# wanxinjin/Pontryagin-Differentiable-Programming

Measured on AMD Instinct MI355X. Metric: trajectories/sec (fwd+Riccati+PDP grad), quadrotor n=13 T=50, higher is better.
Workload: dtype f64

## Files before the change

pontryagin-differentiable-programming_amd/csrc/pdp_fused3_kernels.h:

```cpp
#pragma once
#include "pdp_model_kernels.h"
#include "pdp_wave.h"

#ifndef PDP_F3_GAIN_AHEAD
#define PDP_F3_GAIN_AHEAD 3
#endif
#ifndef PDP_F3_ROLLOUT_LANES
#define PDP_F3_ROLLOUT_LANES 0
#endif

namespace pdp {

#ifdef PDP_PHASE_TIMING
__device__ long long g_rb_stamp[16];
#endif

template <class Mdl, int XW = 0>
struct Fused3Layout {
    using L = FusedLayout<Mdl>;
    static constexpr int NX = Mdl::NX, NU = Mdl::NU, NP = Mdl::NP;
    static constexpr int NCB = 1 + Mdl::PATHA_NCONST + Mdl::PATHB_NCONST, NCF = 1 + Mdl::FWD_NCONST, NCFIN = 1 + Mdl::FIN_NCONST;
    static constexpr int NA = Mdl::PATHA_NVAR, NB = Mdl::PATHB_NVAR > 16 ? Mdl::PATHB_NVAR : 16;
    static constexpr int CB0 = NA + NB;
    static constexpr int BSTRIDE = (CB0 + NCB) | 1;
// ... 79 lines not shown
    long long ts[12]; int nts = 0; long long twait = 0, tw0 = 0;
    const long long rt0 = __builtin_amdgcn_s_memrealtime();
    for (int i = 0; i < 12; ++i) ts[i] = 0;
#define F3_STAMP() ts[nts++] = __builtin_readcyclecounter()
#define F3_W0() tw0 = __builtin_readcyclecounter()
#define F3_W1() twait += __builtin_readcyclecounter() - tw0
#else
#define F3_STAMP()
#define F3_W0()
#define F3_W1()
#endif
    F3_STAMP();

    if (runner) {
        __builtin_amdgcn_s_setprio(3);
        {
            double th0[NP], pc0[Mdl::NPC];
            load_theta<Mdl>(theta, b, tb, th0);
            Mdl::precompute(th0, pc0);
            if (lane == 0) {
#pragma unroll
                for (int i = 0; i < NP; ++i) par[i] = th0[i];
#pragma unroll
                for (int i = 0; i < Mdl::NPC; ++i) par[NP + i] = pc0[i];
            }
            wg_signal(fl + 0, 1);
        }
        double xTr[NX];
        if (given) {
#pragma unroll
            for (int i = 0; i < NX; ++i) xTr[i] = xb[T * NX + i];
        } else {
            double* us = pool;
            for (int i = lane; i < T * NU; i += 64) us[i] = ub[i];
            PDP_F3_PAR();
            double xc[NX], xn[NX], uc[NU];
#pragma unroll
            for (int i = 0; i < NX; ++i) xc[i] = x0[(int64_t)b * NX + i];
            if (lane == 0) {
#pragma unroll
                for (int i = 0; i < NX; ++i) xb[i] = xc[i];
            }
            wave_lds_sync();
            const auto rsX = PDP_BUF_RSRC(xb, (T + 1) * NX * 8);
            const unsigned xvoff = lane == 0 ? 0u : BUF_OOB;
            double un[NU];
#pragma unroll
            for (int i = 0; i < NU; ++i) un[i] = us[i];
#if PDP_F3_ROLLOUT_LANES
            double xs[NX];
#pragma unroll
            for (int i = 0; i < NX; ++i) xs[i] = 0.0;
            for (int tb_ = 0; tb_ < T; tb_ += 64) {
                const int nb = min(64, T - tb_);
                for (int tl_ = 0; tl_ < nb; ++tl_) {
                    const int t = tb_ + tl_, tn = t + 1 < T ? t + 1 : t;
#pragma unroll
                    for (int i = 0; i < NU; ++i) { uc[i] = un[i]; un[i] = us[tn * NU + i]; }
                    Mdl::dyn(xc, uc, th, pc, xn);
                    const bool mine = lane == tl_;
#pragma unroll
                    for (int i = 0; i < NX; ++i) { xc[i] = xn[i]; xs[i] = mine ? xn[i] : xs[i]; }
                }
                const unsigned vo = lane < nb ? (unsigned)(lane * NX) * 8u : BUF_OOB;
                const unsigned so = (unsigned)((tb_ + 1) * NX) * 8u;
#pragma unroll
                for (int i = 0; i + 1 < NX; i += 2) buf_store_f64x2(rsX, so, vo + 8u * i, xs[i], xs[i + 1]);
                if constexpr (NX & 1) buf_store_f64(rsX, so, vo + 8u * (NX - 1), xs[NX - 1]);
            }
#else
            for (int t = 0; t < T; ++t) {
                const int tn = t + 1 < T ? t + 1 : t;
#pragma unroll
                for (int i = 0; i < NU; ++i) { uc[i] = un[i]; un[i] = us[tn * NU + i]; }
                Mdl::dyn(xc, uc, th, pc, xn);
#pragma unroll
                for (int i = 0; i < NX; ++i) xc[i] = xn[i];
                {
                    const unsigned so = (unsigned)((t + 1) * NX) * 8u;
#pragma unroll
                    for (int i = 0; i + 1 < NX; i += 2) buf_store_f64x2(rsX, so, xvoff + 8u * i, xn[i], xn[i + 1]);
                    if constexpr (NX & 1) buf_store_f64(rsX, so, xvoff + 8u * (NX - 1), xn[NX - 1]);
                }
            }
#endif
#pragma unroll
            for (int i = 0; i < NX; ++i) xTr[i] = xc[i];
        }
        wg_signal(fl + 0, 2);
        F3_STAMP();

        bool ok = true;
        d4 P, W2;
        {
            if (lane == 0) fin[0] = 0.0;
            for (int i_ = lane; i_ < Mdl::FIN_NCONST; i_ += 64) fin[1 + i_] = Mdl::fin_const(i_);
            if (lane == 0) {
                PDP_F3_PAR();
                PackedSink s{fin + F3::NCFIN};
                Mdl::eval_fin(xTr, nullptr, nullptr, th, pc, s);
            }
            wave_lds_sync();
            Gather gP, gW;
            make_gather(gP, lane, F3::NCFIN, 0, [](int r, int c) { return (r < NX && c < NX) ? Mdl::fin_code(0, r * NX + c) : -1; });
            make_gather(gW, lane, F3::NCFIN, 0, [](int r, int c) { return (r < NX && c >= M && c < M + NP) ? Mdl::fin_code(1, r * NP + (c - M)) : -1; });
            P = gather_tile(fin, gP, 0);
            W2 = gather_tile(fin, gW, 0);
        }
        F3_STAMP();

        {
            constexpr int NA = F3::NA, NCA = Mdl::PATHA_NCONST;
            auto codeA = [](int mat, int i) { return Mdl::patha_code(mat, i); };
            auto codeB = [](int mat, int i) { int c = Mdl::pathb_code(mat, i); return c >= 0 ? c + NA : (c == -1 ? -1 : c - NCA); };
            RowGather gF, gY, gHxx, gHX, gHU, gGr, gHux;
            make_row_gather(gF, lane, F3::CB0, [&](int r, int c) { return (r < NX && c < NX) ? codeA(0, r * NX + c) : -1; });
            make_row_gather(gY, lane, F3::CB0, [&](int r, int c) {
                return r >= NX ? -1 : (c < M ? codeA(1, r * NU + c) : (c < M + NP ? codeA(2, r * NP + (c - M)) : -1)); });
            make_row_gather(gGr, lane, F3::CB0, [&](int r, int c) { return (r < NX && (c & 3) < NU) ? codeA(1, r * NU + (c & 3)) : -1; });
            make_row_gather(gHux, lane, F3::CB0, [&](int r, int c) { return (r < M && c < NX) ? codeB(1, c * NU + r) : -1; });
            make_row_gather(gHxx, lane, F3::CB0, [&](int r, int c) { return (r < NX && c < NX) ? codeB(0, r * NX + c) : -1; });
            make_row_gather(gHX, lane, F3::CB0, [&](int r, int c) {
                return r >= NX ? -1 : (c < M ? codeB(1, r * NU + c) : (c < M + NP ? codeB(2, r * NP + (c - M)) : -1)); });
            make_row_gather(gHU, lane, F3::CB0, [&](int r, int c) {
                return r >= M ? -1 : (c < M ? codeB(3, r * NU + c) : (c < M + NP ? codeB(4, r * NP + (c - M)) : -1)); });
            const TileMapBytes mK = make_tile_map_sink(NU, NX, NX, 0, 0, lane, GSZ0 - 1), mIK = make_tile_map_sink(NU, NP, NP, 0, M, lane, NU * NP);
            constexpr int RSZ = oc_riccati_doubles<Mdl>();
            [[maybe_unused]] const BufMap mRP = f3_store_map(NX, NX, NX, 0, lane), mRW = f3_store_map(NX, NP, NP, M, lane);
            [[maybe_unused]] const auto rsR = PDP_BUF_RSRC(FM::RIC && riccati ? riccati + (int64_t)b * T * RSZ : ws_gain, FM::RIC && riccati ? (int64_t)T * RSZ * 8 : 0);
            [[maybe_unused]] const PredMaps<Mdl> pm(lane);
            [[maybe_unused]] const bool precPW = FM::RIC && prec && !(flags & PDP_OC_RECORD_PRIMAL);
            [[maybe_unused]] const auto rsPR = PDP_BUF_RSRC(precPW ? (void*)(prec + (int64_t)b * T * PredRec<Mdl>::SIZE) : (void*)ws_gain, precPW ? (int64_t)T * PredRec<Mdl>::SIZE * 4 : 0);
            constexpr int RB = 8 * BS;
            for (int g = 0; g < nchunk; ++g) {
                int t0, cnt;
                bchunk(g, t0, cnt);
                const double* pb = pool + (g & 1) * F3::BUF;
                F3_W0();
                wg_wait_ge(fl + 2, g + 1);
                F3_W1();
                int tl = cnt - 1;
                const double* r0 = pb + (tl - 1) * BS;
                RowRun rF = row_run_at(gF, r0), rY = row_run_at(gY, r0), rHxx = row_run_at(gHxx, r0), rHX = row_run_at(gHX, r0), rHU = row_run_at(gHU, r0),
                     rGr = row_run_at(gGr, r0), rHux = row_run_at(gHux, r0);
                auto move_all = [&](int bytes) {
                    row_move(rF, bytes); row_move(rY, bytes); row_move(rHxx, bytes); row_move(rHX, bytes); row_move<1>(rHU, bytes); row_move(rGr, bytes); row_move<1>(rHux, bytes);
                };
                d4 Fa = row_read(rF, RB), Ya = row_read(rY, RB), Fb = z, Yb = z;
                auto bstep = [&](int tl, unsigned imm, const d4 Fc, const d4 Yc, d4& Fn, d4& Yn) {
                    const int t = t0 + tl;
#ifdef PDP_PHASE_TIMING_FINE
                    if (blockIdx.x == 0 && threadIdx.x == 0) g_rb_stamp[9] = __builtin_readcyclecounter();
#endif
                    d4 Hxx = row_read(rHxx, imm), HX2 = row_read(rHX, imm), HU2 = row_read<1>(rHU, imm), Grep = row_read(rGr, imm), Hux = row_read<1>(rHux, imm);
                    if (tl > 0) { Fn = row_read(rF, imm - RB); Yn = row_read(rY, imm - RB); }
                    RiccatiGains gn;
                    d4 P_old;
                    if constexpr (FM::RIC) {
                        if (riccati) { buf_store(rsR, (unsigned)(t * RSZ) * 8u, mRP, P); buf_store(rsR, (unsigned)(t * RSZ + NX * NX) * 8u, mRW, W2); }
                        if (precPW) { pred_store(rsPR, (unsigned)(t * PredRec<Mdl>::SIZE) * 4u, pm.P, P); pred_store(rsPR, (unsigned)(t * PredRec<Mdl>::SIZE) * 4u, pm.W, W2); }
                    }
                    ok = riccati_backward<M, false>(P, W2, Fc, Yc, Grep, Hxx, HX2, HU2, Hux[0], scratch, lane, NP, gn, P_old) && ok;
                    store_all<1>(gw + t * GSZ, mK, gn.K);
                    store_all<1>(gw + t * GSZ + NX * NU, mIK, gn.IK);
#ifdef PDP_PHASE_TIMING_FINE
                    if (blockIdx.x == 0 && threadIdx.x == 0) { g_rb_stamp[11] = g_rb_stamp[10]; g_rb_stamp[10] = __builtin_readcyclecounter(); }
#endif
                };
                for (; (tl + 1) % U != 0; --tl) { bstep(tl, RB, Fa, Ya, Fb, Yb); Fa = Fb; Ya = Yb; move_all(-RB); }
                move_all(-(U - 1) * RB);
                for (; tl >= U - 1; tl -= U) {
                    static_assert(U == 4, "the group is written out");
                    bstep(tl, (unsigned)(4 * RB), Fa, Ya, Fb, Yb);
                    bstep(tl - 1, (unsigned)(3 * RB), Fb, Yb, Fa, Ya);
                    bstep(tl - 2, (unsigned)(2 * RB), Fa, Ya, Fb, Yb);
                    bstep(tl - 3, (unsigned)(1 * RB), Fb, Yb, Fa, Ya);
                    move_all(-U * RB);
                }
                wg_signal(fl + 3, g + 1);
            }
        }
        bool finite = tile_finite(P) && tile_finite(W2);
        F3_STAMP();

        double acc = 0.0;
        [[maybe_unused]] double lsum = 0.0;
        double dT;
        [[maybe_unused]] bool obsT = true;
        [[maybe_unused]] double sT = 0.0, rhoT = 0.0;
        if constexpr (FM::WLS) { const int li = lane < NX ? lane : 0; wls_slot(dT, sT, xb[T * NX + li], dxb[T * NX + li], wxb[T * NX + li], oc_wls_x(oc_wls(wls...)), rhoT); }
        else if constexpr (FM::COT) dT = lane < NX ? dxb[T * NX + lane] : 0.0;
        else if constexpr (FM::MISS) { const double dd = lane < NX ? dxb[T * NX + lane] : 0.0; obsT = dd == dd; dT = lane < NX ? (obsT ? xb[T * NX + lane] - dd : dd) : 0.0; }
        else dT = lane < NX ? xb[T * NX + lane] - dxb[T * NX + lane] : 0.0;
        d4 X2 = z;
        [[maybe_unused]] d4 Gn = z;
        {
            constexpr int DLX = Mdl::FWD_NVAR, DLU = Mdl::FWD_NVAR + NX;
            [[maybe_unused]] constexpr int DSX = DLU + NU, DSU = DSX + NX;
            RowGather gFT, gGT, gE, gDX, gDU;
            [[maybe_unused]] RowGather gSX, gSU;
            if constexpr (FM::WLS) {
                make_row_gather(gSX, lane, F3::CF0, [](int r, int c) { return (r < NX) ? DSX + r : -1; });
                make_row_gather(gSU, lane, F3::CF0, [](int r, int c) { return (r < M) ? DSU + r : -1; });
            }
            make_row_gather(gFT, lane, F3::CF0, [](int r, int c) { return (r < NX && c < NX) ? Mdl::fwd_code(0, c * NX + r) : -1; });
            make_row_gather(gGT, lane, F3::CF0, [](int r, int c) { return (r < M && c < NX) ? Mdl::fwd_code(1, c * NU + r) : -1; });
            make_row_gather(gE, lane, F3::CF0, [](int r, int c) { return (r < NX && c >= M && c < M + NP) ? Mdl::fwd_code(2, r * NP + (c - M)) : -1; });
            make_row_gather(gDX, lane, F3::CF0, [](int r, int c) { return (r < NX) ? DLX + r : -1; });
            make_row_gather(gDU, lane, F3::CF0, [](int r, int c) { return (r < M) ? DLU + r : -1; });
            const TileMapBytes mKT = to_bytes_sink(make_rep4_map_transposed(NX, NU, NX, lane), GSZ0 - 1), mIK = make_tile_map_sink(NU, NP, NP, 0, M, lane, NU * NP);
#if PDP_F3_GAIN_AHEAD >= 2
            d4 KTs[4], ks[4];
#pragma unroll
            for (int s_ = 0; s_ < 4; ++s_) {
                if (s_ < PDP_F3_GAIN_AHEAD) {
                    const int ts = s_ < T ? s_ : T - 1;
                    KTs[s_] = -load_all<4>(gw + ts * GSZ, mKT);
                    ks[s_] = -load_all<1>(gw + ts * GSZ + NX * NU, mIK);
                } else { KTs[s_] = z; ks[s_] = z; }
            }
#else
            d4 KTn = -load_all<4>(gw, mKT);
            d4 kn = -load_all<1>(gw + NX * NU, mIK);
#endif
            [[maybe_unused]] const BufMap mSX = f3_store_map(NX, NP, NP, M, lane), mSU = f3_store_map(NU, NP, NP, M, lane);
            [[maybe_unused]] const auto rsSX = PDP_BUF_RSRC(dxdp ? dxdp + (int64_t)b * (T + 1) * NX * NP : ws_gain, dxdp ? (int64_t)(T + 1) * NX * NP * 8 : 0);
            [[maybe_unused]] const auto rsSU = PDP_BUF_RSRC(dudp ? dudp + (int64_t)b * T * NU * NP : ws_gain, dudp ? (int64_t)T * NU * NP * 8 : 0);
            [[maybe_unused]] const PredMaps<Mdl> pmf(lane);
            [[maybe_unused]] const auto rsPRf = PDP_BUF_RSRC(FM::RIC && prec ? (void*)(prec + (int64_t)b * T * PredRec<Mdl>::SIZE) : (void*)ws_gain, FM::RIC && prec ? (int64_t)T * PredRec<Mdl>::SIZE * 4 : 0);
            constexpr int RF = 8 * FS;
            static_assert((U & 1) == 0, "the register sets of the unrolled loops alternate: U must be even");
            for (int c = 0; c < nchunkF; ++c) {
                const int g = nchunk + c, t0 = c * chF, cnt = min(chF, T - t0);
                const double* pb = pool + (g & 1) * F3::BUF;
                F3_W0();
                wg_wait_ge(fl + 2, g + 1);
                F3_W1();
                RowRun rFT = row_run_at(gFT, pb), rGT = row_run_at(gGT, pb), rE = row_run_at(gE, pb), rDX = row_run_at(gDX, pb), rDU = row_run_at(gDU, pb);
                [[maybe_unused]] RowRun rSX, rSU;
                if constexpr (FM::WLS) { rSX = row_run_at(gSX, pb); rSU = row_run_at(gSU, pb); }
                auto move_all = [&](int bytes) {
                    row_move(rFT, bytes); row_move<1>(rGT, bytes); row_move(rE, bytes); row_move(rDX, bytes); row_move<1>(rDU, bytes);
                    if constexpr (FM::WLS) { row_move(rSX, bytes); row_move<1>(rSU, bytes); }
                };
                auto fstep = [&](int tl, unsigned imm, const d4 Xc, d4& Xn, const d4 KTc, const d4 kc, d4& KTnx, d4& knx) {
                    const int t = t0 + tl, tnx = (t + PDP_F3_GAIN_AHEAD < T) ? t + PDP_F3_GAIN_AHEAD : T - 1;
                    KTnx = -load_all<4>(gw + tnx * GSZ, mKT);
                    knx = -load_all<1>(gw + tnx * GSZ + NX * NU, mIK);
                    d4 FT = row_read(rFT, imm);
                    d4 GT = row_read<1>(rGT, imm);
                    d4 E2 = row_read(rE, imm);
                    d4 DX = row_read(rDX, imm);
                    d4 DU = row_read<1>(rDU, imm);
                    d4 U2;
                    riccati_forward(KTc, kc, FT, GT, E2, Xc, U2, Xn);
                    d4 Xm = Xc, Um = U2;
                    if constexpr (FM::WLS) {
                        const d4 SX = row_read(rSX, imm), SU = row_read<1>(rSU, imm);
                        Xm = wls_scale(SX, Xc);
                        Um = zero4(); Um[0] = wls_scale(SU, U2)[0];
                    } else
                    mask_step<FM::MISS, 4>(DX, DU, Xc, U2, Xm, Um);
                    if constexpr (FM::GN) Gn = gram_step<false>(Xm, Um, Gn);
                    acc += contract_step(DX, DU, Xm, Um);
                    if constexpr (FM::RIC) {
                        if (dxdp || dudp) {
                            buf_store(rsSX, (unsigned)(t * NX * NP) * 8u, mSX, Xc);
                            buf_store<1>(rsSU, (unsigned)(t * NU * NP) * 8u, mSU, U2);
                        }
                        if (prec) {
                            pred_store(rsPRf, (unsigned)(t * PredRec<Mdl>::SIZE) * 4u, pmf.X, Xn);
                            pred_store<1>(rsPRf, (unsigned)(t * PredRec<Mdl>::SIZE) * 4u, pmf.U, U2);
                        }
                    } else {
                        if (dxdp) store_dense(dxdp + ((int64_t)b * (T + 1) + t) * NX * NP, NX, NP, NP, 0, M, lane, Xc);
                        if (dudp) store_dense(dudp + ((int64_t)b * T + t) * NU * NP, NU, NP, NP, 0, M, lane, U2);
                    }
                };
                d4 Xb;
                int tl = 0;
#if PDP_F3_GAIN_AHEAD >= 2
                static_assert(U == 4 && PDP_F3_GAIN_AHEAD <= 3, "four gain sets rotate through a group of four steps");
                constexpr int A = PDP_F3_GAIN_AHEAD;
                for (; tl + U <= cnt; tl += U) {
                    fstep(tl + 0, (unsigned)(0 * RF), X2, Xb, KTs[0], ks[0], KTs[(0 + A) & 3], ks[(0 + A) & 3]);
                    fstep(tl + 1, (unsigned)(1 * RF), Xb, X2, KTs[1], ks[1], KTs[(1 + A) & 3], ks[(1 + A) & 3]);
                    fstep(tl + 2, (unsigned)(2 * RF), X2, Xb, KTs[2], ks[2], KTs[(2 + A) & 3], ks[(2 + A) & 3]);
                    fstep(tl + 3, (unsigned)(3 * RF), Xb, X2, KTs[3], ks[3], KTs[(3 + A) & 3], ks[(3 + A) & 3]);
                    move_all(U * RF);
                }
                for (; tl < cnt; ++tl) {
                    fstep(tl, 0u, X2, Xb, KTs[0], ks[0], KTs[A], ks[A]);
                    X2 = Xb;
#pragma unroll
                    for (int s_ = 0; s_ < A; ++s_) { KTs[s_] = KTs[s_ + 1]; ks[s_] = ks[s_ + 1]; }
                    move_all(RF);
                }
#else
                d4 KTb, kb;
                for (; tl + U <= cnt; tl += U) {
#pragma unroll
                    for (int j = 0; j < U; ++j) {
                        if (j & 1) fstep(tl + j, (unsigned)(j * RF), Xb, X2, KTb, kb, KTn, kn);
                        else fstep(tl + j, (unsigned)(j * RF), X2, Xb, KTn, kn, KTb, kb);
                    }
                    move_all(U * RF);
                }
                for (; tl < cnt; ++tl) { fstep(tl, 0u, X2, Xb, KTn, kn, KTb, kb); X2 = Xb; KTn = KTb; kn = kb; move_all(RF); }
#endif
                wg_signal(fl + 3, g + 1);
            }
        }
        F3_STAMP();
        wave_lds_sync();
        if (lane < NX) {
// ... 207 lines not shown
```

pontryagin-differentiable-programming_amd/csrc/pdp_riccati.h:

```cpp
#pragma once
#include "pdp_tile.h"

namespace pdp {

constexpr int RICCATI_SCRATCH = 272 + 272 + 64;

PDP_DEV void tile_to_lds17(double* s, const d4 v, int lane) {
#pragma unroll
    for (int r = 0; r < 4; ++r) s[tile_row(lane, r) * 17 + tile_col(lane)] = v[r];
}
PDP_DEV d4 tile_from_lds17_transposed(const double* s, int lane) {
    d4 v;
#pragma unroll
    for (int r = 0; r < 4; ++r) v[r] = s[tile_col(lane) * 17 + tile_row(lane, r)];
    return v;
}

struct RiccatiGains {
    d4 KT;
    d4 K;
    d4 IK;
    d4 Z;
    double Zrep;
    d4 Qux;
    bool pd;
};

template <int M>
PDP_DEV bool posdef_small(const double* a) {
    if constexpr (M == 1) return a[0] > 0.0;
    else if constexpr (M == 2) return a[0] > 0.0 && a[0] * a[3] - a[1] * a[2] > 0.0;
    else {
        const double d2 = a[0] * a[4] - a[1] * a[3];
        const double d3 = a[0] * (a[4] * a[8] - a[5] * a[7]) - a[1] * (a[3] * a[8] - a[5] * a[6]) + a[2] * (a[3] * a[7] - a[4] * a[6]);
        return a[0] > 0.0 && d2 > 0.0 && d3 > 0.0;
    }
}

#ifndef PDP_RB_T
#define PDP_RB_T(i)
#endif
template <int M, bool WANT_KT = true, bool HUX_FROM_HX2 = false, bool WANT_PD = false>
PDP_DEV bool riccati_backward(d4& P, d4& W0, const d4 Ft, const d4 Y2, const d4 Grep, const d4 Hxx, const d4 HX2, const d4 HU2, double Hux0,
                              double* scratch, int lane, int p0, RiccatiGains& g, d4& P_old_out) {
    const d4 z = zero4();
    if constexpr (HUX_FROM_HX2) tile_to_lds17(scratch, HX2, lane);
    PDP_RB_T(0);
    d4 PF = mma_tn(P, Ft, z);
    d4 PY2 = mma_tn(P, Y2, W0);
    PDP_RB_T(1);
    d4 FY = mma_tn(Ft, PY2, HX2);
    d4 Q2 = z;
    Q2[0] = mma4_tn(Grep, PY2, HU2[0]);
    PDP_RB_T(2);
    if constexpr (HUX_FROM_HX2) {
        wave_lds_sync();
        Hux0 = ((lane >> 4) < M) ? scratch[(lane & 15) * 17 + (lane >> 4)] : 0.0;
    }
    d4 Qux = z;
    Qux[0] = mma4_tn(Grep, PF, Hux0);
    d4 Pn = mma_tn(Ft, PF, Hxx);
    P_old_out = P;
    PDP_RB_T(3);
    const int row = lane >> 4, col = lane & 15;
    d4 Z = z;
    double Zrep = 0.0;
    bool ok = true;
    if constexpr (M == 4) {
        scratch[544 + lane] = Q2[0];
        wave_lds_sync();
        PDP_RB_T(4);
        const int i = row, j = col & 3;
        const int r0 = (i == 0) ? 1 : 0, r1 = (i <= 1) ? 2 : 1, r2 = (i <= 2) ? 3 : 2;
        const int c0 = (j == 0) ? 1 : 0, c1 = (j <= 1) ? 2 : 1, c2 = (j <= 2) ? 3 : 2;
        const double* q = scratch + 544;
        const double m00 = q[r0 * 16 + c0], m01 = q[r0 * 16 + c1], m02 = q[r0 * 16 + c2];
        const double m10 = q[r1 * 16 + c0], m11 = q[r1 * 16 + c1], m12 = q[r1 * 16 + c2];
        const double m20 = q[r2 * 16 + c0], m21 = q[r2 * 16 + c1], m22 = q[r2 * 16 + c2];
        double cof = m00 * (m11 * m22 - m12 * m21) - m01 * (m10 * m22 - m12 * m20) + m02 * (m10 * m21 - m11 * m20);
        cof = ((i + j) & 1) ? -cof : cof;
        const double ac = Q2[0] * cof;
        const double t0 = readlane_f64(ac, 0), t1 = readlane_f64(ac, 1), t2 = readlane_f64(ac, 2), t3 = readlane_f64(ac, 3);
        const double det = (t0 + t1) + (t2 + t3), mag = (fabs(t0) + fabs(t1)) + (fabs(t2) + fabs(t3));
        if constexpr (WANT_PD) {
            const double a00 = readlane_f64(Q2[0], 0), a01 = readlane_f64(Q2[0], 1), a10 = readlane_f64(Q2[0], 16), a11 = readlane_f64(Q2[0], 17);
            g.pd = a00 > 0.0 && a00 * a11 - a01 * a10 > 0.0 && readlane_f64(cof, 51) > 0.0 && det > 0.0;
        }
        if (fabs(det) > COFACTOR4_GUARD * mag && fabs(det) <= 1.7e308) {
            double rdet = __builtin_amdgcn_rcp(det);
            rdet = fma(fma(-det, rdet, 1.0), rdet, rdet);
            Zrep = cof * rdet;
        } else {
            double a[16], ai[16];
#pragma unroll
            for (int ii = 0; ii < 4; ++ii)
#pragma unroll
                for (int jj = 0; jj < 4; ++jj) a[ii * 4 + jj] = readlane_f64(Q2[0], 16 * ii + jj);
            ok = inverse_small<4>(a, ai);
            double zz = 0.0;
#pragma unroll
            for (int ii = 0; ii < 4; ++ii)
#pragma unroll
                for (int jj = 0; jj < 4; ++jj) zz = (row == ii && (col & 3) == jj) ? ai[jj * 4 + ii] : zz;
            Zrep = zz;
        }
    } else {
        double a[M * M], ai[M * M];
#pragma unroll
        for (int i = 0; i < M; ++i)
#pragma unroll
            for (int j = 0; j < M; ++j) a[i * M + j] = readlane_f64(Q2[0], 16 * i + j);
        ok = inverse_small_fast<M>(a, ai);
        if constexpr (WANT_PD) g.pd = posdef_small<M>(a);
        double zz = 0.0;
#pragma unroll
        for (int i = 0; i < M; ++i)
#pragma unroll
            for (int j = 0; j < M; ++j) zz = (row == i && (col & 3) == j) ? ai[j * M + i] : zz;
        Zrep = zz;
    }
    Z[0] = (col < 4) ? Zrep : 0.0;
    PDP_RB_T(5);
    d4 K = z;
    K[0] = mma4_blk(Zrep, Qux[0], 0.0);
    g.IK = z;
    g.IK[0] = mma4_blk(Zrep, Q2[0], 0.0);
    if constexpr (WANT_KT) g.KT = mma_tn_r0(Qux, Z, z);
    g.K = K;
    g.Z = Z;
    g.Zrep = Zrep;
    g.Qux = Qux;
    P = mms_tn_r0(Qux, K, Pn);
    tile_to_lds17(scratch + 272, P, lane);
    PDP_RB_T(6);
    d4 Wn = mms_tn_r0(Qux, g.IK, FY);
    W0 = keep_cols(Wn, M, M + p0, lane);
    g.IK = keep_cols(g.IK, M, M + p0, lane);
    wave_lds_sync();
    PDP_RB_T(7);
    P = 0.5 * (P + tile_from_lds17_transposed(scratch + 272, lane));
    PDP_RB_T(8);
    return ok;
}

template <int CTRL>
PDP_DEV double dpp_mov_f64(double v) {
    const int lo = __builtin_amdgcn_update_dpp(0, __double2loint(v), CTRL, 0xf, 0xf, false);
    const int hi = __builtin_amdgcn_update_dpp(0, __double2hiint(v), CTRL, 0xf, 0xf, false);
    return __hiloint2double(hi, lo);
}
template <int M, bool WANT_PD = true>
PDP_DEV bool riccati_backward_aug(d4& P, const d4 Ft, const double Gblk, const d4 Grep, const d4 Hxx, const double HU0, const double Hux0, double* scratch, int lane,
                                  RiccatiGains& g) {
    const d4 z = zero4();
    d4 PF = mma_tn(P, Ft, z);
    const double PGb = mma4_tn(P, Grep, 0.0);
    d4 Q2 = z;
    {
        double q = mma4_blk(Gblk, PGb, HU0);
        q += dpp_mov_f64<0x128>(q);
        q += dpp_mov_f64<0x124>(q);
        Q2[0] = q;
    }
    d4 Qux = z;
    Qux[0] = mma4_tn(Grep, PF, Hux0);
    d4 Pn = mma_tn(Ft, PF, Hxx);
    const int row = lane >> 4, col = lane & 15;
    double Zrep = 0.0;
    bool ok = true;
    if constexpr (M == 4) {
        scratch[544 + lane] = Q2[0];
        wave_lds_sync();
        const int i = row, j = col & 3;
        const int r0 = (i == 0) ? 1 : 0, r1 = (i <= 1) ? 2 : 1, r2 = (i <= 2) ? 3 : 2;
        const int c0 = (j == 0) ? 1 : 0, c1 = (j <= 1) ? 2 : 1, c2 = (j <= 2) ? 3 : 2;
        const double* q = scratch + 544;
        const double m00 = q[r0 * 16 + c0], m01 = q[r0 * 16 + c1], m02 = q[r0 * 16 + c2];
        const double m10 = q[r1 * 16 + c0], m11 = q[r1 * 16 + c1], m12 = q[r1 * 16 + c2];
        const double m20 = q[r2 * 16 + c0], m21 = q[r2 * 16 + c1], m22 = q[r2 * 16 + c2];
        double cof = m00 * (m11 * m22 - m12 * m21) - m01 * (m10 * m22 - m12 * m20) + m02 * (m10 * m21 - m11 * m20);
        cof = ((i + j) & 1) ? -cof : cof;
        const double ac = Q2[0] * cof;
        const double t0 = readlane_f64(ac, 0), t1 = readlane_f64(ac, 1), t2 = readlane_f64(ac, 2), t3 = readlane_f64(ac, 3);
        const double det = (t0 + t1) + (t2 + t3), mag = (fabs(t0) + fabs(t1)) + (fabs(t2) + fabs(t3));
        if constexpr (WANT_PD) {
            const double a00 = readlane_f64(Q2[0], 0), a01 = readlane_f64(Q2[0], 1), a10 = readlane_f64(Q2[0], 16), a11 = readlane_f64(Q2[0], 17);
            g.pd = a00 > 0.0 && a00 * a11 - a01 * a10 > 0.0 && readlane_f64(cof, 51) > 0.0 && det > 0.0;
        }
        if (fabs(det) > COFACTOR4_GUARD * mag && fabs(det) <= 1.7e308) {
            double rdet = __builtin_amdgcn_rcp(det);
            rdet = fma(fma(-det, rdet, 1.0), rdet, rdet);
            Zrep = cof * rdet;
        } else {
            double a[16], ai[16];
#pragma unroll
            for (int ii = 0; ii < 4; ++ii)
#pragma unroll
// ... 55 lines not shown
```

pontryagin-differentiable-programming_amd/csrc/pdp_tile.h:

```cpp
#pragma once
#include <hip/hip_runtime.h>
#include <stdint.h>

typedef double d4 __attribute__((ext_vector_type(4)));

#define PDP_DEV __device__ __forceinline__

namespace pdp {

PDP_DEV int tile_row(int lane, int r) { return (lane >> 4) + 4 * r; }
PDP_DEV int tile_col(int lane) { return lane & 15; }

PDP_DEV d4 zero4() { d4 z = {0.0, 0.0, 0.0, 0.0}; return z; }

PDP_DEV d4 mma_tn(const d4 x, const d4 y, d4 c) {
    c = __builtin_amdgcn_mfma_f64_16x16x4f64(x[0], y[0], c, 0, 0, 0);
    c = __builtin_amdgcn_mfma_f64_16x16x4f64(x[1], y[1], c, 0, 0, 0);
    c = __builtin_amdgcn_mfma_f64_16x16x4f64(x[2], y[2], c, 0, 0, 0);
    c = __builtin_amdgcn_mfma_f64_16x16x4f64(x[3], y[3], c, 0, 0, 0);
    return c;
}
PDP_DEV d4 mma_tn_r0(const d4 x, const d4 y, d4 c) {
    return __builtin_amdgcn_mfma_f64_16x16x4f64(x[0], y[0], c, 0, 0, 0);
}
PDP_DEV d4 mms_tn_r0(const d4 x, const d4 y, d4 c) {
    return __builtin_amdgcn_mfma_f64_16x16x4f64(-x[0], y[0], c, 0, 0, 0);
}

PDP_DEV double mma4_blk(double xrep, double y, double c) { return __builtin_amdgcn_mfma_f64_4x4x4f64(xrep, y, c, 0, 0, 0); }
PDP_DEV double mma4_tn(const d4 xrep, const d4 y, double c) {
    c = mma4_blk(xrep[0], y[0], c);
    c = mma4_blk(xrep[1], y[1], c);
    c = mma4_blk(xrep[2], y[2], c);
    c = mma4_blk(xrep[3], y[3], c);
    return c;
}

template <bool TRANS>
PDP_DEV d4 load_dense(const double* __restrict__ M, int R, int C, int ld, int roff, int coff, int lane) {
    d4 v;
#pragma unroll
    for (int r = 0; r < 4; ++r) {
        int row = tile_row(lane, r) - roff, col = tile_col(lane) - coff;
        bool ok = TRANS ? (row >= 0 && row < C && col >= 0 && col < R) : (row >= 0 && row < R && col >= 0 && col < C);
        double x = 0.0;
        if (ok) x = TRANS ? M[col * ld + row] : M[row * ld + col];
        v[r] = x;
    }
    return v;
}
PDP_DEV void store_dense(double* __restrict__ M, int R, int C, int ld, int roff, int coff, int lane, const d4 v) {
#pragma unroll
    for (int r = 0; r < 4; ++r) {
        int row = tile_row(lane, r) - roff, col = tile_col(lane) - coff;
        if (row >= 0 && row < R && col >= 0 && col < C) M[row * ld + col] = v[r];
    }
}
struct TileMap {
    int off[4];
};
PDP_DEV TileMap make_tile_map(int R, int C, int ld, int roff, int coff, int lane) {
    TileMap m;
#pragma unroll
    for (int r = 0; r < 4; ++r) {
        int row = tile_row(lane, r) - roff, col = tile_col(lane) - coff;
        m.off[r] = (row >= 0 && row < R && col >= 0 && col < C) ? row * ld + col : -1;
    }
    return m;
}
template <bool TRANS>
PDP_DEV TileMap make_dense_map(int R, int C, int ld, int roff, int coff, int lane) {
    if (!TRANS) return make_tile_map(R, C, ld, roff, coff, lane);
    TileMap m;
#pragma unroll
    for (int r = 0; r < 4; ++r) {
        int row = tile_row(lane, r) - roff, col = tile_col(lane) - coff;
        m.off[r] = (row >= 0 && row < C && col >= 0 && col < R) ? col * ld + row : -1;
    }
    return m;
}
PDP_DEV TileMap make_rep4_map(int R, int C, int ld, int lane) {
    TileMap m;
#pragma unroll
    for (int r = 0; r < 4; ++r) {
        const int row = tile_row(lane, r), c = tile_col(lane) & 3;
        m.off[r] = (row < R && c < C) ? row * ld + c : -1;
    }
    return m;
}
PDP_DEV TileMap make_rep4_map_transposed(int R, int C, int ld, int lane) {
    TileMap m;
#pragma unroll
    for (int r = 0; r < 4; ++r) {
        const int row = tile_row(lane, r), c = tile_col(lane) & 3;
        m.off[r] = (row < R && c < C) ? c * ld + row : -1;
    }
    return m;
}
template <int NR = 4>
PDP_DEV d4 load_map(const double* __restrict__ base, const TileMap& m) {
    d4 v = zero4();
#pragma unroll
    for (int r = 0; r < NR; ++r) { const int o = m.off[r]; const double x = base[o >= 0 ? o : 0]; v[r] = o >= 0 ? x : 0.0; }
    return v;
}
template <int NR = 4>
PDP_DEV void store_map(double* __restrict__ base, const TileMap& m, const d4 v) {
#pragma unroll
    for (int r = 0; r < NR; ++r) if (m.off[r] >= 0) base[m.off[r]] = v[r];
}
struct TileMapBytes { unsigned off[4]; };
PDP_DEV TileMapBytes to_bytes_sink(const TileMap& m, int sink) {
    TileMapBytes b;
#pragma unroll
    for (int r = 0; r < 4; ++r) b.off[r] = 8u * (unsigned)(m.off[r] < 0 ? sink : m.off[r]);
    return b;
}
PDP_DEV TileMapBytes make_tile_map_sink(int R, int C, int ld, int roff, int coff, int lane, int sink) {
    TileMap m = make_tile_map(R, C, ld, roff, coff, lane);
    TileMapBytes b;
#pragma unroll
    for (int r = 0; r < 4; ++r) b.off[r] = 8u * (unsigned)(m.off[r] < 0 ? sink : m.off[r]);
    return b;
}
template <int NR = 4>
PDP_DEV void store_all(double* __restrict__ base, const TileMapBytes& m, const d4 v) {
#pragma unroll
    for (int r = 0; r < NR; ++r) {
        unsigned o = m.off[r];
        asm("" : "+v"(o));
        *(double*)((char*)base + o) = v[r];
    }
}
template <int NR = 4>
PDP_DEV d4 load_all(const double* __restrict__ base, const TileMapBytes& m) {
    d4 v = zero4();
#pragma unroll
    for (int r = 0; r < NR; ++r) {
        unsigned o = m.off[r];
        asm("" : "+v"(o));
        v[r] = *(const double*)((const char*)base + o);
    }
    return v;
}
PDP_DEV d4 keep_cols(const d4 v, int c0, int c1, int lane) {
    int col = tile_col(lane);
    return (col >= c0 && col < c1) ? v : zero4();
}
PDP_DEV bool tile_finite(const d4 v) {
    bool ok = true;
#pragma unroll
    for (int r = 0; r < 4; ++r) ok = ok && (fabs(v[r]) <= 1.7e308);
    return ok;
}

PDP_DEV void wave_lds_sync() { asm volatile("s_waitcnt lgkmcnt(0)" ::: "memory"); }

PDP_DEV double pdp_tanh(double x) {
    const double ax = fmin(fabs(x), 20.0);
    const double d = exp(2.0 * ax) + 1.0;
    double r = __builtin_amdgcn_rcp(d);
    r = fma(fma(-d, r, 1.0), r, r);
    r = fma(fma(-d, r, 1.0), r, r);
    const double t = fma(-2.0, r, 1.0);
    return x != x ? x : copysign(t, x);
}

PDP_DEV double readlane_f64(double v, int src) {
    int lo = __builtin_amdgcn_readlane(__double2loint(v), src);
    int hi = __builtin_amdgcn_readlane(__double2hiint(v), src);
    return __hiloint2double(hi, lo);
}

template <int M>
PDP_DEV bool inverse_small(const double* a_in, double* inv) {
    double a[M][M], b[M][M];
#pragma unroll
    for (int i = 0; i < M; ++i)
#pragma unroll
        for (int j = 0; j < M; ++j) { a[i][j] = a_in[i * M + j]; b[i][j] = (i == j) ? 1.0 : 0.0; }
    bool ok = true;
#pragma unroll
    for (int k = 0; k < M; ++k) {
#pragma unroll
        for (int i = k + 1; i < M; ++i) {
            bool sw = fabs(a[i][k]) > fabs(a[k][k]);
#pragma unroll
            for (int j = 0; j < M; ++j) {
                double t = a[k][j], s = a[i][j];
                a[k][j] = sw ? s : t; a[i][j] = sw ? t : s;
                t = b[k][j]; s = b[i][j];
                b[k][j] = sw ? s : t; b[i][j] = sw ? t : s;
            }
        }
        double piv = a[k][k];
        ok = ok && (fabs(piv) > 1e-300) && (fabs(piv) <= 1.7e308);
        double ip = 1.0 / piv;
#pragma unroll
        for (int j = 0; j < M; ++j) { a[k][j] *= ip; b[k][j] *= ip; }
#pragma unroll
        for (int i = 0; i < M; ++i) {
            if (i == k) continue;
            double f = a[i][k];
#pragma unroll
            for (int j = 0; j < M; ++j) { a[i][j] -= f * a[k][j]; b[i][j] -= f * b[k][j]; }
        }
    }
#pragma unroll
    for (int i = 0; i < M; ++i)
#pragma unroll
        for (int j = 0; j < M; ++j) inv[i * M + j] = b[i][j];
    return ok;
}

constexpr double COFACTOR4_GUARD = 1e-2;
template <int M>
constexpr double ADJUGATE_GUARD = (M >= 3) ? 1e-4 : 1e-10;

template <int M>
PDP_DEV bool inverse_small_fast(const double* a, double* inv) {
    double dprod = 1.0;
#pragma unroll
    for (int i = 0; i < M; ++i) dprod *= a[i * M + i];
    double det, c[M * M];
    if constexpr (M == 1) {
        det = a[0]; c[0] = 1.0;
    } else if constexpr (M == 2) {
        det = a[0] * a[3] - a[1] * a[2];
        c[0] = a[3]; c[1] = -a[1]; c[2] = -a[2]; c[3] = a[0];
    } else if constexpr (M == 3) {
        c[0] = a[4] * a[8] - a[5] * a[7]; c[1] = a[2] * a[7] - a[1] * a[8]; c[2] = a[1] * a[5] - a[2] * a[4];
        c[3] = a[5] * a[6] - a[3] * a[8]; c[4] = a[0] * a[8] - a[2] * a[6]; c[5] = a[2] * a[3] - a[0] * a[5];
        c[6] = a[3] * a[7] - a[4] * a[6]; c[7] = a[1] * a[6] - a[0] * a[7]; c[8] = a[0] * a[4] - a[1] * a[3];
        det = a[0] * c[0] + a[1] * c[3] + a[2] * c[6];
    } else {
        const double s0 = a[0] * a[5] - a[4] * a[1], s1 = a[0] * a[6] - a[4] * a[2], s2 = a[0] * a[7] - a[4] * a[3];
        const double s3 = a[1] * a[6] - a[5] * a[2], s4 = a[1] * a[7] - a[5] * a[3], s5 = a[2] * a[7] - a[6] * a[3];
        const double c5 = a[10] * a[15] - a[14] * a[11], c4 = a[9] * a[15] - a[13] * a[11], c3 = a[9] * a[14] - a[13] * a[10];
        const double c2 = a[8] * a[15] - a[12] * a[11], c1 = a[8] * a[14] - a[12] * a[10], c0 = a[8] * a[13] - a[12] * a[9];
        det = s0 * c5 - s1 * c4 + s2 * c3 + s3 * c2 - s4 * c1 + s5 * c0;
        c[0] = a[5] * c5 - a[6] * c4 + a[7] * c3;   c[1] = -a[1] * c5 + a[2] * c4 - a[3] * c3;
        c[2] = a[13] * s5 - a[14] * s4 + a[15] * s3; c[3] = -a[9] * s5 + a[10] * s4 - a[11] * s3;
        c[4] = -a[4] * c5 + a[6] * c2 - a[7] * c1;  c[5] = a[0] * c5 - a[2] * c2 + a[3] * c1;
        c[6] = -a[12] * s5 + a[14] * s2 - a[15] * s1; c[7] = a[8] * s5 - a[10] * s2 + a[11] * s1;
        c[8] = a[4] * c4 - a[5] * c2 + a[7] * c0;   c[9] = -a[0] * c4 + a[1] * c2 - a[3] * c0;
        c[10] = a[12] * s4 - a[13] * s2 + a[15] * s0; c[11] = -a[8] * s4 + a[9] * s2 - a[11] * s0;
        c[12] = -a[4] * c3 + a[5] * c1 - a[6] * c0; c[13] = a[0] * c3 - a[1] * c1 + a[2] * c0;
        c[14] = -a[12] * s3 + a[13] * s1 - a[14] * s0; c[15] = a[8] * s3 - a[9] * s1 + a[10] * s0;
    }
    if (!(fabs(det) > ADJUGATE_GUARD<M> * fabs(dprod)) || !(fabs(det) <= 1.7e308)) return inverse_small<M>(a, inv);
    double id = __builtin_amdgcn_rcp(det);
    id = fma(fma(-det, id, 1.0), id, id);
#pragma unroll
    for (int i = 0; i < M * M; ++i) inv[i] = c[i] * id;
    return true;
}

PDP_DEV double sum_over_rowgroups(double v) {
    v += __shfl_xor(v, 16, 64);
    v += __shfl_xor(v, 32, 64);
    return v;
}
PDP_DEV double wave_sum(double v) {
#pragma unroll
    for (int o = 32; o > 0; o >>= 1) v += __shfl_xor(v, o, 64);
    return v;
}

}
```

Baseline: 11.65 million.

## Add hand-scheduled Riccati backward step for M=4 with interleaved MFMA and cofactor inverse

Adds a specialized Riccati backward routine for 4 controls that pins the instruction order with sched_group_barrier and sched_barrier. It splits the MFMA chains so the 4x4 Quu cofactor inverse, the LDS transpose and the lane reductions overlap with independent MFMA work. The row reads are also reordered so the loads needed first are issued first. The intent is to hide MFMA and LDS latency on the serial backward pass. The cost is a fragile hand schedule and a weaker LDS ordering fence (compiler-only) in place of an lgkmcnt wait.

```diff
diff --git a/pontryagin-differentiable-programming_amd/csrc/pdp_fused3_kernels.h b/pontryagin-differentiable-programming_amd/csrc/pdp_fused3_kernels.h
--- a/pontryagin-differentiable-programming_amd/csrc/pdp_fused3_kernels.h
+++ b/pontryagin-differentiable-programming_amd/csrc/pdp_fused3_kernels.h
@@ -255,7 +255,8 @@
 #ifdef PDP_PHASE_TIMING_FINE
                     if (blockIdx.x == 0 && threadIdx.x == 0) g_rb_stamp[9] = __builtin_readcyclecounter();
 #endif
-                    d4 Hxx = row_read(rHxx, imm), HX2 = row_read(rHX, imm), HU2 = row_read<1>(rHU, imm), Grep = row_read(rGr, imm), Hux = row_read<1>(rHux, imm);
+                    __builtin_amdgcn_sched_barrier(0);
+                    d4 HU2 = row_read<1>(rHU, imm), Grep = row_read(rGr, imm), Hux = row_read<1>(rHux, imm), Hxx = row_read(rHxx, imm), HX2 = row_read(rHX, imm);
                     if (tl > 0) { Fn = row_read(rF, imm - RB); Yn = row_read(rY, imm - RB); }
                     RiccatiGains gn;
                     d4 P_old;
@@ -263,7 +264,7 @@
                         if (riccati) { buf_store(rsR, (unsigned)(t * RSZ) * 8u, mRP, P); buf_store(rsR, (unsigned)(t * RSZ + NX * NX) * 8u, mRW, W2); }
                         if (precPW) { pred_store(rsPR, (unsigned)(t * PredRec<Mdl>::SIZE) * 4u, pm.P, P); pred_store(rsPR, (unsigned)(t * PredRec<Mdl>::SIZE) * 4u, pm.W, W2); }
                     }
-                    ok = riccati_backward<M, false>(P, W2, Fc, Yc, Grep, Hxx, HX2, HU2, Hux[0], scratch, lane, NP, gn, P_old) && ok;
+                    ok = riccati_backward<M, false, false, false, true>(P, W2, Fc, Yc, Grep, Hxx, HX2, HU2, Hux[0], scratch, lane, NP, gn, P_old) && ok;
                     store_all<1>(gw + t * GSZ, mK, gn.K);
                     store_all<1>(gw + t * GSZ + NX * NU, mIK, gn.IK);
 #ifdef PDP_PHASE_TIMING_FINE
diff --git a/pontryagin-differentiable-programming_amd/csrc/pdp_riccati.h b/pontryagin-differentiable-programming_amd/csrc/pdp_riccati.h
--- a/pontryagin-differentiable-programming_amd/csrc/pdp_riccati.h
+++ b/pontryagin-differentiable-programming_amd/csrc/pdp_riccati.h
@@ -40,9 +40,104 @@
 #ifndef PDP_RB_T
 #define PDP_RB_T(i)
 #endif
-template <int M, bool WANT_KT = true, bool HUX_FROM_HX2 = false, bool WANT_PD = false>
+PDP_DEV bool riccati_backward_sched4(d4& P, d4& W0, const d4 Ft, const d4 Y2, const d4 Grep, const d4 Hxx, const d4 HX2, const d4 HU2, const double Hux0,
+                                     double* scratch, int lane, int p0, RiccatiGains& g, d4& P_old_out) {
+    const d4 z = zero4();
+    const int row = lane >> 4, col = lane & 15;
+    P_old_out = P;
+    d4 PY2 = mma_tn(P, Y2, W0);
+    __builtin_amdgcn_sched_group_barrier(0x008, 1, 0);
+    __builtin_amdgcn_sched_group_barrier(0x100, 8, 0);
+    __builtin_amdgcn_sched_group_barrier(0x008, 1, 0);
+    __builtin_amdgcn_sched_group_barrier(0x100, 8, 0);
+    __builtin_amdgcn_sched_group_barrier(0x008, 1, 0);
+    __builtin_amdgcn_sched_group_barrier(0x100, 8, 0);
+    __builtin_amdgcn_sched_group_barrier(0x008, 1, 0);
+    __builtin_amdgcn_sched_barrier(0);
+    d4 PF = __builtin_amdgcn_mfma_f64_16x16x4f64(P[0], Ft[0], z, 0, 0, 0);
+    __builtin_amdgcn_sched_barrier(0);
+    d4 Q2 = z;
+    Q2[0] = mma4_tn(Grep, PY2, HU2[0]);
+    __builtin_amdgcn_sched_barrier(0);
+    PF = __builtin_amdgcn_mfma_f64_16x16x4f64(P[1], Ft[1], PF, 0, 0, 0);
+    __builtin_amdgcn_sched_barrier(0);
+    scratch[544 + lane] = Q2[0];
+    wave_lds_order();
+    const int i = row, j = col & 3;
+    const int r0 = (i == 0) ? 1 : 0, r1 = (i <= 1) ? 2 : 1, r2 = (i <= 2) ? 3 : 2;
+    const int c0 = (j == 0) ? 1 : 0, c1 = (j <= 1) ? 2 : 1, c2 = (j <= 2) ? 3 : 2;
+    const double* q = scratch + 544;
+    const double m00 = q[r0 * 16 + c0], m01 = q[r0 * 16 + c1], m02 = q[r0 * 16 + c2];
+    const double m10 = q[r1 * 16 + c0], m11 = q[r1 * 16 + c1], m12 = q[r1 * 16 + c2];
+    const double m20 = q[r2 * 16 + c0], m21 = q[r2 * 16 + c1], m22 = q[r2 * 16 + c2];
+    __builtin_amdgcn_sched_barrier(0);
+    PF = __builtin_amdgcn_mfma_f64_16x16x4f64(P[2], Ft[2], PF, 0, 0, 0);
+    PF = __builtin_amdgcn_mfma_f64_16x16x4f64(P[3], Ft[3], PF, 0, 0, 0);
+    __builtin_amdgcn_sched_barrier(0);
+    double cof = m00 * (m11 * m22 - m12 * m21) - m01 * (m10 * m22 - m12 * m20) + m02 * (m10 * m21 - m11 * m20);
+    cof = ((i + j) & 1) ? -cof : cof;
+    const double ac = Q2[0] * cof;
+    const double t0 = readlane_f64(ac, 0), t1 = readlane_f64(ac, 1), t2 = readlane_f64(ac, 2), t3 = readlane_f64(ac, 3);
+    const double det = (t0 + t1) + (t2 + t3), mag = (fabs(t0) + fabs(t1)) + (fabs(t2) + fabs(t3));
+    double rdet = __builtin_amdgcn_rcp(det);
+    __builtin_amdgcn_sched_barrier(0);
+    d4 Qux = z;
+    Qux[0] = mma4_tn(Grep, PF, Hux0);
+    __builtin_amdgcn_sched_barrier(0);
+    rdet = fma(fma(-det, rdet, 1.0), rdet, rdet);
+    asm volatile("" : "+v"(rdet));
+    d4 Pn = mma_tn(Ft, PF, Hxx);
+    double Zrep = cof * rdet;
+    bool ok = true;
+    if (__builtin_expect(!(fabs(det) > COFACTOR4_GUARD * mag && fabs(det) <= 1.7e308), 0)) {
+        double a[16], ai[16];
+#pragma unroll
+        for (int ii = 0; ii < 4; ++ii)
+#pragma unroll
+            for (int jj = 0; jj < 4; ++jj) a[ii * 4 + jj] = readlane_f64(Q2[0], 16 * ii + jj);
+        ok = inverse_small<4>(a, ai);
+        double zz = 0.0;
+#pragma unroll
+        for (int ii = 0; ii < 4; ++ii)
+#pragma unroll
+            for (int jj = 0; jj < 4; ++jj) zz = (row == ii && (col & 3) == jj) ? ai[jj * 4 + ii] : zz;
+        Zrep = zz;
+    }
+    d4 Z = z;
+    Z[0] = (col < 4) ? Zrep : 0.0;
+    d4 K = z;
+    K[0] = mma4_blk(Zrep, Qux[0], 0.0);
+    g.IK = z;
+    g.IK[0] = mma4_blk(Zrep, Q2[0], 0.0);
+    g.K = K;
+    g.Z = Z;
+    g.Zrep = Zrep;
+    g.Qux = Qux;
+    P = mms_tn_r0(Qux, K, Pn);
+    __builtin_amdgcn_sched_barrier(0);
+    d4 FY = __builtin_amdgcn_mfma_f64_16x16x4f64(Ft[0], PY2[0], HX2, 0, 0, 0);
+    __builtin_amdgcn_sched_barrier(0);
+    tile_to_lds17(scratch + 272, P, lane);
+    wave_lds_order();
+    const d4 Pt = tile_from_lds17_transposed(scratch + 272, lane);
+    __builtin_amdgcn_sched_barrier(0);
+    FY = __builtin_amdgcn_mfma_f64_16x16x4f64(Ft[1], PY2[1], FY, 0, 0, 0);
+    FY = __builtin_amdgcn_mfma_f64_16x16x4f64(Ft[2], PY2[2], FY, 0, 0, 0);
+    FY = __builtin_amdgcn_mfma_f64_16x16x4f64(Ft[3], PY2[3], FY, 0, 0, 0);
+    d4 Wn = mms_tn_r0(Qux, g.IK, FY);
+    __builtin_amdgcn_sched_barrier(0);
+    P = 0.5 * (P + Pt);
+    __builtin_amdgcn_sched_barrier(0);
+    W0 = keep_cols(Wn, 4, 4 + p0, lane);
+    g.IK = keep_cols(g.IK, 4, 4 + p0, lane);
+    return ok;
+}
+
+template <int M, bool WANT_KT = true, bool HUX_FROM_HX2 = false, bool WANT_PD = false, bool SCHED = false>
 PDP_DEV bool riccati_backward(d4& P, d4& W0, const d4 Ft, const d4 Y2, const d4 Grep, const d4 Hxx, const d4 HX2, const d4 HU2, double Hux0,
                               double* scratch, int lane, int p0, RiccatiGains& g, d4& P_old_out) {
+    if constexpr (SCHED && M == 4 && !WANT_KT && !HUX_FROM_HX2 && !WANT_PD)
+        return riccati_backward_sched4(P, W0, Ft, Y2, Grep, Hxx, HX2, HU2, Hux0, scratch, lane, p0, g, P_old_out);
     const d4 z = zero4();
     if constexpr (HUX_FROM_HX2) tile_to_lds17(scratch, HX2, lane);
     PDP_RB_T(0);
diff --git a/pontryagin-differentiable-programming_amd/csrc/pdp_tile.h b/pontryagin-differentiable-programming_amd/csrc/pdp_tile.h
--- a/pontryagin-differentiable-programming_amd/csrc/pdp_tile.h
+++ b/pontryagin-differentiable-programming_amd/csrc/pdp_tile.h
@@ -155,6 +155,7 @@
 }
 
 PDP_DEV void wave_lds_sync() { asm volatile("s_waitcnt lgkmcnt(0)" ::: "memory"); }
+PDP_DEV void wave_lds_order() { asm volatile("" ::: "memory"); }
 
 PDP_DEV double pdp_tanh(double x) {
     const double ax = fmin(fabs(x), 20.0);
diff --git a/probes/record_fused3_sched_golden.py b/probes/record_fused3_sched_golden.py
--- /dev/null
+++ b/probes/record_fused3_sched_golden.py
@@ -0,0 +1,23 @@
+import os
+import sys
+
+import numpy as np
+
+ROOT = os.path.dirname(os.path.dirname(os.path.abspath(__file__)))
+sys.path.insert(0, ROOT)
+sys.path.insert(0, os.path.join(ROOT, "tests"))
+import fused3_sched_common as fc
+
+commit, path = sys.argv[1], sys.argv[2]
+rec = {"seed": np.int64(fc.SEED), "commit": np.array(commit)}
+t5 = None
+for name in fc.CASES:
+    out = fc.run_case(name, given=t5)
+    if name == "T5":
+        t5 = (out["x"], out["lam"])
+    for k, v in out.items():
+        rec["%s/%s" % (name, k)] = v
+    print(name, {k: v.shape for k, v in out.items()}, "status", out["status"].tolist())
+os.makedirs(os.path.dirname(os.path.abspath(path)), exist_ok=True)
+np.savez_compressed(path, **rec)
+print("wrote %s (%d bytes)" % (path, os.path.getsize(path)))
```

New measurement: 12.04 million (median of 6 runs). +3.3%, better.
